# dynatrace-oss/index4j

Hardware: AMD Instinct MI355X
Metric: patterns/sec + LF-steps/sec, 1M x 8-char count() on 256 MiB log index (higher is better)
Workload: dtype int32; 1 GPU; count() batch of 1048576 random 8-char patterns per GPU on 256 MiB synthetic log text, sampleRate=32 (BASELINE.json configs[1]); 4 distinct batches rotate through the timed loop; image=expanded, text_chars=268435456, patterns_per_gpu=1048576, pattern_len=8, batches=4, count_checksum=151883111733, patterns_checked_vs_oracle=0, parallelism=dp1

## Files before the change

### include/fmx.h

```cpp
#ifndef FMX_H
#define FMX_H

#include <stddef.h>
#include <stdint.h>

#ifdef __cplusplus
extern "C" {
#endif

typedef struct fmx_index fmx_index;

#define FMX_OK 0
#define FMX_E_ARG (-1)
#define FMX_E_ALPHABET (-2)
#define FMX_E_FORMAT (-3)
#define FMX_E_VERSION (-4)
#define FMX_E_NO_DEVICE (-5)
#define FMX_E_HIP (-6)
#define FMX_E_NOMEM (-7)
#define FMX_E_UNSUPPORTED (-8)

#define FMX_ST_OK 0
#define FMX_ST_NOT_ENABLED 1
#define FMX_ST_POS_NEGATIVE 2
#define FMX_ST_STOP_TOO_LONG 3
#define FMX_ST_DEST_TOO_SMALL 4
#define FMX_ST_POS_TOO_LONG 5
#define FMX_ST_DEST_SIZE_ZERO 6
#define FMX_ST_NO_BOUNDARY 7
#define FMX_ST_DOES_NOT_FIT 8
#define FMX_ST_JAVA_AIOOBE 9
#define FMX_ST_TOO_MANY_RANGES 10


int fmx_build(const uint16_t *text, int32_t n, int32_t sample_rate, int enable_extract, fmx_index **out);
int fmx_build_on_device(const uint16_t *text, int32_t n, int32_t sample_rate, int enable_extract, int device,
                        fmx_index **out, int32_t *rounds, int64_t *rows_sorted, double *stage_seconds);
double fmx_build_wavelet_seconds(const fmx_index *idx);

int fmx_suffix_table_info(const fmx_index *idx, int32_t *chars, int64_t *bytes);

int fmx_window_cells_info(const fmx_index *idx, int64_t *bytes);
int fmx_locate_rows_info(const fmx_index *idx, int64_t *bytes, int64_t *replay_rows);
int fmx_resident_bytes(const fmx_index *idx, int64_t *image, int64_t *suffix_table, int64_t *window_directory);

int fmx_load(const uint8_t *ser, size_t len, fmx_index **out);

int fmx_save(const fmx_index *idx, int framed, uint8_t **buf, size_t *len);
int fmx_save_key_order_modelled(const fmx_index *idx);
void fmx_free_buffer(uint8_t *buf);
void fmx_free(fmx_index *idx);

int32_t fmx_input_length(const fmx_index *idx);
int32_t fmx_alphabet_length(const fmx_index *idx);
int32_t fmx_sample_rate(const fmx_index *idx);
int32_t fmx_extract_enabled(const fmx_index *idx);


int fmx_blob(const fmx_index *idx, const uint8_t **blob, size_t *len);
int fmx_to_device(fmx_index *idx, int device);
int fmx_attach_device_blob(void *device_blob, size_t len, int device, fmx_index **out);
void *fmx_device_blob(const fmx_index *idx, size_t *len);

// ... 282 lines not shown
```

### index4j_amd/_lib.py

```python
import ctypes as C
import os

_HERE = os.path.dirname(os.path.abspath(__file__))
LIB_PATH = os.environ.get("FMX_LIBRARY") or os.path.join(_HERE, "libfmx.so")

OK = 0
E_ARG, E_ALPHABET, E_FORMAT, E_VERSION, E_NO_DEVICE, E_HIP, E_NOMEM, E_UNSUPPORTED = -1, -2, -3, -4, -5, -6, -7, -8

ST_OK = 0
ST_NOT_ENABLED = 1
ST_POS_NEGATIVE = 2
ST_STOP_TOO_LONG = 3
ST_DEST_TOO_SMALL = 4
ST_POS_TOO_LONG = 5
ST_DEST_SIZE_ZERO = 6
ST_NO_BOUNDARY = 7
ST_DOES_NOT_FIT = 8
ST_JAVA_AIOOBE = 9
ST_TOO_MANY_RANGES = 10

SYMBOLS = [
    "fmx_build", "fmx_build_on_device", "fmx_build_wavelet_seconds", "fmx_suffix_table_info", "fmx_window_cells_info", "fmx_locate_rows_info", "fmx_load", "fmx_save", "fmx_save_key_order_modelled", "fmx_free_buffer", "fmx_free",
    "fmx_input_length", "fmx_alphabet_length", "fmx_sample_rate", "fmx_extract_enabled",
    "fmx_blob", "fmx_to_device", "fmx_attach_device_blob", "fmx_device_blob", "fmx_host_register", "fmx_host_unregister",
    "fmx_count_batch", "fmx_locate_batch", "fmx_locate_all_batch", "fmx_match_lines_batch", "fmx_match_query_batch", "fmx_count_class_batch", "fmx_locate_all_class_batch", "fmx_match_query_class_batch", "fmx_match_sequence_batch", "fmx_match_sequence_class_batch", "fmx_field_values_batch", "fmx_field_values_class_batch", "fmx_field_values_where_batch", "fmx_field_values_where_class_batch", "fmx_line_histogram_batch", "fmx_line_histogram_class_batch", "fmx_hit_histogram_where_batch", "fmx_hit_histogram_where_class_batch", "fmx_line_bounds_batch", "fmx_extract_packed_batch", "fmx_line_text_batch", "fmx_extract_packed_last_redo", "fmx_extract_batch", "fmx_extract_boundary_batch",
    "fmx_count_batch_dev", "fmx_count_plan_dev", "fmx_count_ordered_dev", "fmx_count_batch_is_planned", "fmx_batch_policy", "fmx_locate_batch_dev", "fmx_locate_all_ranges_dev", "fmx_locate_all_fill_dev", "fmx_line_table_build", "fmx_line_table_info", "fmx_line_bounds_batch_dev", "fmx_lines_of_hits_scratch_bytes", "fmx_lines_of_hits_dev", "fmx_hit_lines_geometry", "fmx_query_lines_scratch_bytes", "fmx_query_lines_of_hits_dev", "fmx_sequence_lines_scratch_bytes", "fmx_sequence_lines_of_hits_dev", "fmx_values_of_hits_scratch_bytes", "fmx_values_of_hits_dev", "fmx_values_fill_dev", "fmx_hits_in_lines_scratch_bytes", "fmx_hits_in_lines_dev", "fmx_lines_histogram_scratch_bytes", "fmx_hits_histogram_scratch_bytes", "fmx_lines_histogram_dev", "fmx_hits_histogram_dev", "fmx_class_ranges_scratch_bytes", "fmx_class_ranges_count_dev", "fmx_class_ranges_fill_dev", "fmx_class_hit_offsets_scratch_bytes", "fmx_class_hit_offsets_dev", "fmx_class_fold_status_dev", "fmx_extract_packed_scratch_bytes", "fmx_extract_packed_offsets_dev", "fmx_extract_packed_fill_dev", "fmx_extract_batch_dev", "fmx_extract_boundary_batch_dev",
    "fmx_locate_extract_batch", "fmx_locate_lines_batch", "fmx_locate_extract_batch_dev", "fmx_locate_lines_batch_dev",
    "fmx_count_segments", "fmx_locate_segments", "fmx_count_segments_dev", "fmx_locate_segments_dev", "fmx_count_locate_segments_dev",
    "fmx_count_locate_segments", "fmx_resident_bytes",
    "fmx_replicate", "fmx_device_of", "fmx_shard_range", "fmx_count_batch_multi", "fmx_locate_batch_multi", "fmx_extract_batch_multi",
    "fmx_extract_boundary_batch_multi", "fmx_count_locate_segments_multi", "fmx_count_batch_multi_dev",
    "fmx_count_locate_segments_multi_dev", "fmx_multi_synchronize",
    "fmx_wavelet_build", "fmx_wavelet_rank_batch", "fmx_wavelet_inverse_select_batch",
    "fmx_rrr_build", "fmx_rrr_rank_ones_batch", "fmx_rrr_access_batch", "fmx_rrr_rank_ones_batch_dev", "fmx_rrr_access_batch_dev",
    "fmx_sa_build", "fmx_sa_load", "fmx_sa_save", "fmx_sa_get", "fmx_sa_hash_code", "fmx_sa_count_batch", "fmx_sa_locate_batch",
    "fmx_sa_count_batch_dev", "fmx_sa_locate_batch_dev", "fmx_bwt",
    "fmx_convert_byte_pattern", "fmx_status_message", "fmx_status_kind", "fmx_last_error", "fmx_release_scratch", "fmx_device_count", "fmx_set_option",
    "fmx_synth_log", "fmx_synth_log_multichar", "fmx_synth_patterns",
]


def _load():
    if not os.path.exists(LIB_PATH):
        raise ImportError(
            "index4j_amd: %s is missing - build it with `python -c 'import __graft_entry__ as g; g.build()'` "
            "or `make -C index4j_amd/csrc` (hipcc, gfx950). There is no CPU fallback." % LIB_PATH
        )
    L = C.CDLL(LIB_PATH)
    vp, i32, u16, u64 = C.c_void_p, C.c_int32, C.c_uint16, C.c_uint64
    P = C.POINTER
    sz = C.c_size_t
    L.fmx_build.argtypes = [vp, i32, i32, C.c_int, P(vp)]
    L.fmx_build_on_device.argtypes = [vp, i32, i32, C.c_int, C.c_int, P(vp), P(i32), P(C.c_int64), P(C.c_double)]
    L.fmx_build_wavelet_seconds.argtypes = [vp]
    L.fmx_build_wavelet_seconds.restype = C.c_double
    L.fmx_suffix_table_info.argtypes = [vp, P(i32), P(C.c_int64)]
    L.fmx_window_cells_info.argtypes = [vp, P(C.c_int64)]
    L.fmx_locate_rows_info.argtypes = [vp, P(C.c_int64), P(C.c_int64)]
    L.fmx_load.argtypes = [vp, sz, P(vp)]
    L.fmx_save.argtypes = [vp, C.c_int, P(vp), P(sz)]
    L.fmx_save_key_order_modelled.argtypes = [vp]
    L.fmx_batch_policy.argtypes = [vp, C.c_int, C.c_int64]
    L.fmx_free_buffer.argtypes = [vp]
    L.fmx_free_buffer.restype = None
    L.fmx_free.argtypes = [vp]
    L.fmx_free.restype = None
    for name in ("fmx_input_length", "fmx_alphabet_length", "fmx_sample_rate", "fmx_extract_enabled"):
        getattr(L, name).argtypes = [vp]
        getattr(L, name).restype = i32
    L.fmx_blob.argtypes = [vp, P(vp), P(sz)]
    L.fmx_to_device.argtypes = [vp, C.c_int]
    L.fmx_attach_device_blob.argtypes = [vp, sz, C.c_int, P(vp)]
    L.fmx_device_blob.argtypes = [vp, P(sz)]
    L.fmx_device_blob.restype = vp
    L.fmx_host_register.argtypes = [vp, sz]
    L.fmx_host_unregister.argtypes = [vp]
    L.fmx_count_batch.argtypes = [vp, vp, vp, i32, vp, vp, vp]
    L.fmx_locate_batch.argtypes = [vp, vp, vp, i32, i32, vp, i32, vp, vp, vp]
    L.fmx_extract_batch.argtypes = [vp, vp, vp, i32, vp, i32, i32, vp, vp, vp]
# ... 150 lines not shown
```

### index4j_amd/csrc/fmx_api.cpp

```cpp
#include "../../include/fmx.h"
#include "fmx_device.hpp"
#include "fmx_build_stage.hpp"
#include "fmx_hit_values.hpp"
#include "fmx_model.hpp"
#include "fmx_options.hpp"
#include "fmx_plan.hpp"
#include "fmx_sa_index.hpp"

#include <hip/hip_runtime.h>

#include <immintrin.h>

#include <atomic>
#include <chrono>
#include <climits>
#include <condition_variable>
#include <deque>
#include <cstdio>
#include <cstdlib>
#include <cstring>
#include <map>
#include <memory>
#include <mutex>
#include <new>
// ... 1216 lines not shown
    if (key_bits == 8 && idx->hdr.wt_sigma <= fmx::kOrder1MaxSigma &&
        fmx::order1_lds_bytes(fmx::kPlanDefaultBins, idx->hdr.wt_sigma) <= fmx::kPlanCodesLdsMax) {
        void *d_o1 = nullptr;
        const size_t bytes = (size_t)idx->hdr.wt_sigma * idx->hdr.wt_sigma * 2 * sizeof(float);
        if (hipMalloc(&d_o1, bytes) == hipSuccess) {
            if (k_launch_suffix_order1(idx, idx->dev, static_cast<float *>(d_o1), nullptr) == 0 &&
                hipStreamSynchronize(nullptr) == hipSuccess) {
                idx->d_suffix_order1 = d_o1;
                idx->dev.suffix_order1 = static_cast<const float *>(d_o1);
            } else {
                (void)hipFree(d_o1);
            }
        }
    }
}

int fmx_suffix_table_info(const fmx_index *idx, int32_t *chars, int64_t *bytes) {
    return guarded([&]() -> int {
    if (!idx || idx->sa) return fail(FMX_E_ARG, "not an FM-index handle");
    if (chars) *chars = idx->dev.suffix_table ? idx->dev.suffix_chars : 0;
    if (bytes) *bytes = (int64_t)idx->suffix_table_bytes;
    return FMX_OK;
    });
}

int fmx_blob(const fmx_index *idx_c, const uint8_t **blob, size_t *len) {
    return guarded([&]() -> int {
    fmx_index *idx = const_cast<fmx_index *>(idx_c);
    if (!idx || !blob || !len) return fail(FMX_E_ARG, "null argument");
    int rc = ensure_blob(idx);
    if (rc) return rc;
    *blob = idx->blob.data();
    *len = idx->blob.size();
    return FMX_OK;
    });
}

int fmx_to_device(fmx_index *idx, int device) {
    return guarded([&]() -> int {
    if (!idx) return fail(FMX_E_ARG, "null index");
    if (idx->sa) {
        std::string err;
        const int rc = fmx::sa_to_device(*idx->sa, device, err);
        return rc ? fail(rc, err) : FMX_OK;
    }
    int rc = ensure_blob(idx);
// ... 3000 lines not shown
```

### index4j_amd/csrc/fmx_kernels.hip

```cpp
#include <atomic>
#include <cstring>

#include <hip/hip_runtime.h>

#include "fmx_device.hpp"
#include "fmx_options.hpp"
#include "fmx_plan.hpp"

#if !defined(FMX_KNS)
#define FMX_KNS fmx
#endif

namespace FMX_KNS {
using namespace fmx;
#include "fmx_kernel_api.hpp"

#if FMX_COMPACT
#define FMX_KERNEL(BLOCK) __global__ __launch_bounds__(BLOCK)
#else
#define FMX_KERNEL(BLOCK) __global__ __launch_bounds__(BLOCK) __attribute__((amdgpu_waves_per_eu(8, 8)))
#endif
#ifndef FMX_WALK_WAVES
#define FMX_WALK_WAVES 8
#endif
// ... 1402 lines not shown
template <int kBlock>
FMX_KERNEL(kBlock) void k_rrr_access(DevIndex ix, const int32_t *__restrict__ positions, int32_t n,
                                     uint8_t *__restrict__ out, int32_t *__restrict__ status_out) {
    __shared__ uint16_t s_inv[kInvEntries];
    stage_inverse_table(s_inv, ix.inv_global);
    const RrrView v = rrr_view_from(Quad{ix.sampled.off_rec, ix.sampled.off_bits, (uint32_t)ix.sampled.length, (uint32_t)ix.sampled.total_ones});
    const int64_t stride = (int64_t)gridDim.x * kBlock;
    for (int64_t q = (int64_t)blockIdx.x * kBlock + threadIdx.x; q < n; q += stride) {
        int status = ST_OK;
        const bool bit = rrr_access(ix.base, v, s_inv, positions[q], status);
        out[q] = status ? 0 : (bit ? 1 : 0);
        if (status_out) status_out[q] = status;
    }
}



struct PlanTables {
    const int16_t *s_map;
    const float2 *s_o1;
    const int32_t *s_c;
    bool o1;
    int sigma, below, fine_shift, bins;
};
__device__ __forceinline__ bool plan_uses_order1(const DevIndex &ix, const SortShape &sh, int code_bits, int bins, size_t extra_lds) {
    return code_bits == 8 && sh.sa_key == 2 && ix.suffix_order1 != nullptr && ix.wt_sigma <= kOrder1MaxSigma &&
           order1_lds_bytes(bins, ix.wt_sigma) + extra_lds <= kPlanCodesLdsMax;
}
__device__ __forceinline__ PlanTables plan_tables_stage(const DevIndex &ix, const SortShape &sh, int16_t *s_map, uint32_t *after, bool o1) {
    PlanTables t;
    t.sigma = ix.wt_sigma;
    t.bins = 1 << sh.coarse_bits;
    t.below = sh.total_bits - sh.coarse_bits;
    t.fine_shift = t.below > 8 ? t.below - 8 : 0;
    t.o1 = o1;
    for (int i = threadIdx.x; i < 256; i += kTileThreads) s_map[i] = ix.char2code[i];
    float2 *s_o1 = reinterpret_cast<float2 *>(after);
    int32_t *s_c = reinterpret_cast<int32_t *>(s_o1 + (o1 ? t.sigma * t.sigma : 0));
    if (o1) {
        const float2 *src = reinterpret_cast<const float2 *>(ix.suffix_order1);
        for (int i = threadIdx.x; i < t.sigma * t.sigma; i += kTileThreads) s_o1[i] = src[i];
        for (int i = threadIdx.x; i <= t.sigma; i += kTileThreads) s_c[i] = i < ix.n_c ? ix.C[i] : ix.length;
    }
    t.s_map = s_map;
    t.s_o1 = s_o1;
    t.s_c = s_c;
    return t;
}

template <int kCodeBits>
__device__ __forceinline__ Quad plan_record(const DevIndex &ix, const PlanTables &L, const SortShape &sh, const uint16_t *__restrict__ pat,
                                            int32_t beg, int32_t m, const TailWords &tail, uint32_t &bin) {
    const int sigma = L.sigma;
    uint32_t ch[8];
    pattern_tail_chars(tail, pat, beg, m, ch);
    const uint64_t word = pattern_code_word<kCodeBits>(ix, L.s_map, ch, m);
    uint32_t key;
    if (sh.sa_key) {
        key = 0;
        constexpr uint32_t cmask = (1u << kCodeBits) - 1u;
        const int32_t c_last = (int32_t)(word & cmask);
        if (m > 0 && c_last != 0) {
            int32_t start = ix.C[c_last], end = 0, back = 0;
            int len = fm_suffix_len(ix, m);
            if (len > 64 / kCodeBits) len = 64 / kCodeBits;
            if (len >= 2 && kCodeBits == ix.suffix_key_bits && sh.sa_key == 1) {
                const int bits = len * kCodeBits;
                const uint64_t tk = bits >= 64 ? word : (word & ((1ull << bits) - 1ull));
                if ((uint32_t)(tk >> (bits - kCodeBits)) != 0u && tk != kSuffixEmpty) (void)fm_suffix_lookup(ix, tk, len, start, end, back);
            } else if (len >= 2 && L.o1) {
                auto code_at = [&](int j) { return (uint32_t)(word >> (j * kCodeBits)) & cmask; };
                uint32_t x = code_at(len - 1), y = code_at(len - 2);
                if (x >= (uint32_t)sigma) x = 0;
                if (y >= (uint32_t)sigma) y = 0;
                float lo = (float)L.s_c[x ? x : ((uint32_t)c_last < (uint32_t)sigma ? c_last : 0)], width = 0.0f;
                if (x != 0 && y != 0) {
                    float2 fp = L.s_o1[x * sigma + y];
                    if (fp.y > 0.0f) {
                        const float nx = (float)(L.s_c[x + 1] - L.s_c[x]);
                        lo = (float)L.s_c[x] + fp.x * nx;
                        width = fp.y * nx;
                        for (int j = len - 3; j >= 0 && width >= 1.0f; --j) {
                            x = y;
                            y = code_at(j);
                            if (y == 0 || y >= (uint32_t)sigma) break;
                            fp = L.s_o1[x * sigma + y];
                            if (fp.y <= 0.0f) break;
                            lo += width * fp.x;
                            width *= fp.y;
                        }
                    }
                }
                start = (int32_t)lo;
                if (start < 0) start = 0;
                if (start > ix.length) start = ix.length;
            } else if (len >= 2 && kCodeBits == ix.suffix_key_bits) {
                auto code_at = [&](int j) { return (uint32_t)(word >> (j * kCodeBits)) & cmask; };
                uint32_t x = code_at(len - 1), y = code_at(len - 2);
                float lo = (float)ix.C[x ? x : c_last], width = 0.0f;
                int32_t s2 = 0, e2 = 0;
                if (x != 0 && y != 0 && fm_suffix_lookup(ix, (uint64_t)y | ((uint64_t)x << kCodeBits), 2, s2, e2, back)) {
                    lo = (float)s2;
                    width = (float)(e2 - s2);
                    for (int j = len - 3; j >= 0 && width >= 1.0f; --j) {
                        x = y;
                        y = code_at(j);
                        if (y == 0 || !fm_suffix_lookup(ix, (uint64_t)y | ((uint64_t)x << kCodeBits), 2, s2, e2, back)) break;
                        const float cx = (float)ix.C[x], nx = (float)(ix.C[x + 1] - ix.C[x]);
                        lo += width * ((float)s2 - cx) / nx;
                        width *= (float)(e2 - s2) / nx;
                    }
                }
                start = (int32_t)lo;
                if (start < 0) start = 0;
                if (start > ix.length) start = ix.length;
            }
            key = (uint32_t)start;
        }
    } else {
        key = suffix_key(word, kCodeBits, sh.chars, sh.bits);
    }
    const uint32_t lenf = m < 0 ? 0u : ((uint32_t)m < kPlanLongPattern ? (uint32_t)m : kPlanLongPattern);
    Quad q;
    q.x = (uint32_t)word;
    q.y = (uint32_t)(word >> 32);
    q.z = key;
    q.w = lenf | (((key >> L.fine_shift) & ((1u << kFineBits) - 1u)) << 22);
    uint32_t c = key >> L.below;
    if (c >= (uint32_t)L.bins) c = (uint32_t)L.bins - 1u;
    bin = c;
    return q;
}

template <int kCodeBits>
__global__ __launch_bounds__(kTileThreads) void k_plan_codes(DevIndex ix, const uint16_t *__restrict__ pat,
                                                             const int32_t *__restrict__ pat_off, int32_t n,
                                                             SortShape sh, PlanRec *__restrict__ recs,
                                                             uint32_t *__restrict__ ghist, uint32_t *__restrict__ mixed,
                                                             uint32_t epoch) {
    extern __shared__ uint32_t s_hist[];
    __shared__ int16_t s_map[256];
    const int bins = 1 << sh.coarse_bits;
    for (int i = threadIdx.x; i < bins; i += kTileThreads) s_hist[i] = 0;
    const PlanTables L = plan_tables_stage(ix, sh, s_map, s_hist + bins, plan_uses_order1(ix, sh, kCodeBits, bins, 0));
    __syncthreads();
    const int64_t base = (int64_t)blockIdx.x * kTile;
    const int32_t m_first = pat_off[1] - pat_off[0];
    bool differs = false;
    constexpr int kGroup = kTileItems < 4 ? kTileItems : 4;
    for (int k0 = 0; k0 < kTileItems; k0 += kGroup) {
        int32_t beg[kGroup], len[kGroup];
        TailWords tail[kGroup];
#pragma unroll
        for (int k = 0; k < kGroup; ++k) {
            const int64_t p = base + (int64_t)(k0 + k) * kTileThreads + threadIdx.x;
            beg[k] = 0;
            len[k] = -1;
            if (p < n) {
                beg[k] = pat_off[p];
                len[k] = pat_off[p + 1] - beg[k];
            }
        }
#pragma unroll
        for (int k = 0; k < kGroup; ++k) tail[k] = pattern_tail_load(pat, beg[k], len[k]);
#pragma unroll
        for (int k = 0; k < kGroup; ++k) {
            const int64_t p = base + (int64_t)(k0 + k) * kTileThreads + threadIdx.x;
            if (p >= n) continue;
            differs |= len[k] != m_first;
            uint32_t c;
// ... 281 lines not shown
        for (int k = 0; k < 8; ++k) {
            const int i = i0 + k * kTileThreads + (int)threadIdx.x;
            if (cnt[k]) s_cnt[i] = s_scan[i] + got[k];
        }
    }
    __syncthreads();
#pragma unroll
    for (int k = 0; k < kTileItems; ++k) {
        uint32_t slot = 0;
        if constexpr (kFromRange) slot = wave_ticket(&s_cnt[0], bin[k] == 0u);
        if (bin[k] != 0xffffffffu && !(kFromRange && bin[k] == 0u)) slot = atomicAdd(&s_cnt[bin[k]], 1u);
        if (bin[k] != 0xffffffffu) *reinterpret_cast<Quad *>(recs_out + slot) = mine[k];
    }
    __syncthreads();
    if (threadIdx.x == 0) s_last = atomicAdd(ticket, 1u) == gridDim.x - 1 ? 1u : 0u;
    __syncthreads();
    if (s_last) {
        for (int i = threadIdx.x; i < bins; i += kTileThreads) {
            ghist[i] = 0;
            cursor[i] = 0;
        }
        if (threadIdx.x == 0) *ticket = 0;
    }
}

__global__ __launch_bounds__(kFineThreads) void k_plan_fine(PlanRec *__restrict__ recs, int32_t n) {
    constexpr int n_bins = 1 << kFineBits;
    __shared__ uint32_t s_bin[n_bins];
    __shared__ Quad s_rec[kFineWindow];
    for (int i = threadIdx.x; i < n_bins; i += kFineThreads) s_bin[i] = 0;
    __syncthreads();
    const int64_t base = (int64_t)blockIdx.x * kFineWindow;
    Quad r[kFineItems];
    uint32_t bin[kFineItems];
#pragma unroll
    for (int k = 0; k < kFineItems; ++k) {
        const int64_t q = base + (int64_t)k * kFineThreads + threadIdx.x;
        bin[k] = 0xffffffffu;
        if (q < n) {
            r[k] = ld_quad(recs + q);
            bin[k] = r[k].w >> 22;
            r[k].w &= kPlanLongPattern;
        }
    }
#pragma unroll
    for (int k = 0; k < kFineItems; ++k)
// ... 165 lines not shown
    if (options().plan_fused && !fine_pass && n_cu > 0 && tiles <= n_cu) {
        const size_t lds_fused = std::max(lds_codes, (size_t)bins * 8);
        const uint32_t spin_limit = (uint32_t)options().plan_spin_limit.load();
        if (code_bits == 8)
            hipLaunchKernelGGL(k_plan_fused<8>, dim3(tiles), dim3(kTileThreads), lds_fused, st, ix, pat, off, n, sh, ordered, ghist, ticket,
                               ticket + 2, epoch, spin_limit);
        else if (code_bits == 12)
            hipLaunchKernelGGL(k_plan_fused<12>, dim3(tiles), dim3(kTileThreads), (size_t)bins * 8, st, ix, pat, off, n, sh, ordered, ghist,
                               ticket, ticket + 2, epoch, spin_limit);
        else
            hipLaunchKernelGGL(k_plan_fused<16>, dim3(tiles), dim3(kTileThreads), (size_t)bins * 8, st, ix, pat, off, n, sh, ordered, ghist,
                               ticket, ticket + 2, epoch, spin_limit);
    } else {
    if (code_bits == 8)
        hipLaunchKernelGGL(k_plan_codes<8>, dim3(tiles), dim3(kTileThreads), lds_codes, st, ix, pat, off, n, sh, recs,
                           ghist, ticket + 2, epoch);
    else if (code_bits == 12)
        hipLaunchKernelGGL(k_plan_codes<12>, dim3(tiles), dim3(kTileThreads), (size_t)bins * 4, st, ix, pat, off, n, sh, recs,
                           ghist, ticket + 2, epoch);
    else
        hipLaunchKernelGGL(k_plan_codes<16>, dim3(tiles), dim3(kTileThreads), (size_t)bins * 4, st, ix, pat, off, n, sh, recs,
                           ghist, ticket + 2, epoch);
    if (hipError_t e = hipGetLastError(); e != hipSuccess) return (int)e;
    hipLaunchKernelGGL(k_plan_scatter<false>, dim3(tiles), dim3(kTileThreads), (size_t)bins * 8, st, recs, nullptr, nullptr, 0, n, bins,
                       sh.total_bits - sh.coarse_bits, ghist, cursor, ticket, ordered);
    }
    if (options().plan_fine == 2 || (options().plan_fine == 1 && !sh.sa_key))
        hipLaunchKernelGGL(k_plan_fine, dim3((n + kFineWindow - 1) / kFineWindow), dim3(kFineThreads), 0, st, ordered, n);
    plan->recs = ordered;
    plan->redo_list = reinterpret_cast<int32_t *>(recs);
    plan->redo_count = ticket + 8;
    plan->mixed = ticket + 2;
    plan->epoch = epoch;
    plan->n = n;
    plan->code_bits = code_bits;
    plan->shape = sh;
    plan->look_up = ix.look_up;
    plan->sigma = ix.wt_sigma;
    return (int)hipGetLastError();
}

int launch_count(const DevIndex &ix, int n_cu, const uint16_t *pat, const int32_t *off, const CountPlan *plan,
                 bool plan_is_foreign, int32_t n, int32_t *counts, int32_t *lf, int32_t *status, int32_t *range,
                 hipStream_t st) {
    if (n <= 0) return 0;
    const PlanRec *recs = (plan && plan->recs && plan->n == n) ? static_cast<const PlanRec *>(plan->recs) : nullptr;
    CountPlan none;
    const CountPlan &pl = recs ? *plan : none;
// ... 134 lines not shown
    if (n <= 0) return 0;
    const int32_t slots = fm_locate_slots(max_matches, loc_cap);
    const PlanRec *order = nullptr;
    const uint32_t *order_idle = nullptr;
    const size_t need = (ix.rows && !options().rows_order.load()) ? 0 : walk_workspace_bytes(ix, n);
    if (workspace && need != 0 && workspace_bytes >= need && loc_cap > 0) {
        uint8_t *wsb = static_cast<uint8_t *>(workspace);
        uint32_t *ghist = reinterpret_cast<uint32_t *>(wsb);
        uint32_t *cursor = ghist + (1 << kCoarseBitsMax);
        uint32_t *ticket = cursor + (1 << kCoarseBitsMax);
        PlanRec *ordered = reinterpret_cast<PlanRec *>(wsb + kPlanHeadBytes);
        if (!head_is_zero) {
            hipError_t e = hipMemsetAsync(workspace, 0, kPlanHeadBytes, st);
            if (e != hipSuccess) return (int)e;
        }
        int total_bits = 1;
        while (total_bits < 32 && (1ll << total_bits) <= (long long)ix.length) ++total_bits;
        const int coarse_bits = total_bits < options().coarse_bits ? total_bits : (int)options().coarse_bits;
        const int bins = (1 << coarse_bits) + 1, below = total_bits - coarse_bits;
        const int tiles = (n + kTile - 1) / kTile;
        hipLaunchKernelGGL(k_walk_hist, dim3(tiles), dim3(kTileThreads), (size_t)bins * 4, st, range, n, bins, below, taken,
                           max_matches, ghist, nullptr, nullptr, 1);
        if (hipError_t e = hipGetLastError(); e != hipSuccess) return (int)e;
        hipLaunchKernelGGL(k_plan_scatter<true>, dim3(tiles), dim3(kTileThreads), (size_t)bins * 8, st, nullptr, range, taken,
                           max_matches, n, bins, below, ghist, cursor, ticket, ordered);
        if (hipError_t e = hipGetLastError(); e != hipSuccess) return (int)e;
        if (options().walk_fine)
            hipLaunchKernelGGL(k_plan_fine, dim3((n + kFineWindow - 1) / kFineWindow), dim3(kFineThreads), 0, st, ordered, n);
        order = ordered;
        order_idle = ticket + 1;
    }
    if (ix.rows) {
        const int32_t lanes_log2 = fm_rows_lanes_log2(slots);
        FMX_DISPATCH(k_locate_rows, (int64_t)n << lanes_log2, ix, range, n, max_matches, locs, loc_cap, lanes_log2, found, lf, status, taken,
                     order, set_locs, set_base);
        return (int)hipGetLastError();
    }
    const int64_t tickets = (int64_t)n * fm_walk_lanes(slots);
    if (ix.win && options().walk_queue.load() && ix.sample_rate >= 4 && slots >= options().walk_queue_min_slots.load()) {
        const int64_t waves = (tickets + 63) / 64;
        int32_t per = options().walk_queue.load();
        const int32_t chunk = 64 * per;
        int32_t burst = options().walk_burst.load();
        if (burst <= 0) burst = ix.sample_rate / 4 > 2 ? ix.sample_rate / 4 : 2;
        (void)waves;
        FMX_DISPATCH_FORM(k_locate_walk_q, ix, (tickets + per - 1) / per, ix, range, n, max_matches, locs, loc_cap, slots, found, lf, status, taken, order,
                     order_idle, set_locs, set_base, chunk, burst);
        return (int)hipGetLastError();
// ... 88 lines not shown
    const int order_min = options().boundary_order_min;
    if (order_min <= 0 || n < order_min || n > INT32_MAX) return 0;
    return kPlanHeadBytes + (size_t)n * sizeof(PlanRec) + 64;
}

static int launch_position_order(const DevIndex &ix, const int32_t *positions, int32_t n, const int32_t *slot_found, int32_t slots,
                                 void *order_ws, bool head_is_zero, PlanRec *ordered, hipStream_t st) {
    uint8_t *wsb = static_cast<uint8_t *>(order_ws);
    uint32_t *ghist = reinterpret_cast<uint32_t *>(wsb);
    uint32_t *cursor = ghist + (1 << kCoarseBitsMax);
    uint32_t *ticket = cursor + (1 << kCoarseBitsMax);
    if (!head_is_zero) {
        hipError_t e = hipMemsetAsync(order_ws, 0, kPlanHeadBytes, st);
        if (e != hipSuccess) return (int)e;
    }
    int total_bits = 1;
    while (total_bits < 32 && (1ll << total_bits) <= (long long)ix.length) ++total_bits;
    const int coarse_bits = total_bits < options().coarse_bits ? total_bits : (int)options().coarse_bits;
    const int bins = (1 << coarse_bits) + 1, below = total_bits - coarse_bits;
    const int tiles = (n + kTile - 1) / kTile;
    hipLaunchKernelGGL(k_walk_hist, dim3(tiles), dim3(kTileThreads), (size_t)bins * 4, st, nullptr, n, bins, below, nullptr, 0, ghist,
                       positions, slot_found, slots < 1 ? 1 : slots);
    if (hipError_t e = hipGetLastError(); e != hipSuccess) return (int)e;
    hipLaunchKernelGGL(k_plan_scatter<true>, dim3(tiles), dim3(kTileThreads), (size_t)bins * 8, st, nullptr, nullptr, nullptr, 0, n, bins,
                       below, ghist, cursor, ticket, ordered, positions, slot_found, slots < 1 ? 1 : slots);
    if (hipError_t e = hipGetLastError(); e != hipSuccess) return (int)e;
    hipLaunchKernelGGL(k_plan_fine, dim3((n + kFineWindow - 1) / kFineWindow), dim3(kFineThreads), 0, st, ordered, n);
    return (int)hipGetLastError();
}

int launch_extract(const DevIndex &ix, int n_cu, const int32_t *start, const int32_t *stop, int64_t n, uint16_t *dst,
                   int32_t dst_len, int32_t offset, int32_t *out_len, int32_t *lf, int32_t *status,
                   const int32_t *slot_found, int32_t slots, int32_t fixed_len, void *order_ws, size_t order_ws_bytes,
                   bool head_is_zero, hipStream_t st) {
    if (n <= 0) return 0;
    const PlanRec *order = nullptr;
    const size_t order_need = slot_found ? boundary_order_bytes(ix, n) : 0;
    if (order_ws && order_need != 0 && order_ws_bytes >= order_need) {
        PlanRec *ordered = reinterpret_cast<PlanRec *>(static_cast<uint8_t *>(order_ws) + kPlanHeadBytes);
        if (int e = launch_position_order(ix, start, (int32_t)n, slot_found, slots, order_ws, head_is_zero, ordered, st)) return e;
        order = ordered;
    }
    FMX_DISPATCH_WIN(k_extract, ix, n, ix, start, stop, n, dst, dst_len, offset, out_len, lf, status, slot_found, slots, fixed_len, order);
    return (int)hipGetLastError();
}

struct BoundaryShape {
    int block, group, accel;
// ... 156 lines not shown
```

### index4j_amd/csrc/fmx_options.cpp

```cpp
#include "fmx_options.hpp"

#include <string_view>

#include "fmx_model.hpp"

namespace fmx {
namespace {

bool is_block(int v) { return v == 512 || v == 1024; }
bool is_boundary_group(int v) { return v == 0 || v == 1 || v == 2 || v == 4 || v == 8 || v == 16; }
bool is_first_fill(int v) { return v == 0 || v == 2; }
bool is_entry_bytes(int v) { return v == 0 || v == 4 || v == 6; }
bool is_fence_count(int v) { return v >= 0 && v <= 32768 && !(v & (v - 1)); }

using O = Options;
constexpr Accept any = range(INT_MIN, INT_MAX);

constexpr OptionRow kOptions[] = {
    {"block", 512, &O::block, one_of(is_block), "threads per workgroup"},
    {"groups_per_cu", 16, &O::groups_per_cu, range(1, 64), "grid cap: workgroups per CU, the rest grid-stride"},
    {"lds_pad_kb", 0, &O::lds_pad_kb, range(0, 96), "experiment knob: extra dynamic LDS per workgroup (lowers occupancy)"},

    {"sort_min", 16384, &O::sort_min, at_least(0), "batches at least this large are processed in suffix-sorted order (0 = never)"},
    {"sort_bits", 28, &O::sort_bits, range(1, 32), "full key width: floor(sort_bits / bits-per-code) trailing characters"},
// ... 51 lines not shown
    {"host_pipeline_chunk", 262144, &O::host_pipeline_chunk, at_least(65536), "patterns per stage of that pipeline"},
    {"host_mapped", 1, &O::host_mapped, flag(), "every array of a host-buffer count registered -> one launch over the mapped arrays, no copies"},
    {"host_direct_stores", 1, &O::host_direct_stores, flag(), "the pipeline's kernels store results straight into registered arrays"},
    {"host_stage_threads", 0, &O::host_stage_threads, range(0, 64), "host threads that stage a pageable array into pinned memory (0 / 1 = the runtime's own staging)"},

    {"segments_direct", 1, &O::segments_direct, flag(), "0 = every segment's hits staged and appended (A/B)"},
    {"segments_overlap", 1, &O::segments_overlap, flag(), "0 = a segment set's kernels all on the caller's stream (A/B)"},
    {"segments_overlap_min", 262144, &O::segments_overlap_min, at_least(0), "... and only for batches at least this large"},
};
static_assert(sizeof(kOptions) / sizeof(kOptions[0]) == 58, "a new option needs its entry in tests/test_option_ranges.py too");

}

Options::Options() {
    for (const OptionRow &row : kOptions)
        if (row.store.member) (this->*row.store.member).store(row.def);
}

Options &options() {
    static Options instance;
    return instance;
}

const OptionRow *find_option(const char *name) {
    for (const OptionRow &row : kOptions)
        if (std::string_view(row.name) == name) return &row;
    return nullptr;
}

bool OptionRow::set(int value) const {
    if (value < accept.lo || value > accept.hi || (accept.one_of && !accept.one_of(value))) return false;
    if (accept.flag) value = value != 0;
    if (store.member)
        (options().*store.member).store(value);
    else
        store.setter(value);
    return true;
}

}
```

### index4j_amd/csrc/fmx_options.hpp

```cpp
#pragma once

#include <atomic>
#include <climits>

namespace fmx {

constexpr int kCoarseBitsMax = 14;

struct Options {
    std::atomic<int> block, groups_per_cu, lds_pad_kb;
    std::atomic<int> sort_min, sort_bits, coarse_bits, plan_fine, plan_sa_key, plan_sa_min, plan_min_per_string, plan_fused,
        plan_spin_limit, code_bits_12, suffix_table, regroup_by_length, lf_steps_executed_only, count_halve_uniform, count_lean;
    std::atomic<int> walk_pack, walk_queue, walk_queue_min_slots, walk_burst, walk_order_min, walk_fine, rows_order;
    std::atomic<int> boundary_accel, boundary_group, boundary_first_fill, boundary_narrow, boundary_narrow_min, boundary_rounds,
        boundary_order_min;
    std::atomic<int> sb_cache_limit, suffix_table_mb, suffix_table_chars, suffix_table_image_fraction, window_cells,
        window_cells_mb, window_entry_bytes, window_flat_fraction, locate_rows, sa_fences, sa_fence_chars, wavelet_on_device;
    std::atomic<int> host_small_max, host_pipeline_min, host_pipeline_chunk, host_mapped, host_direct_stores, host_stage_threads,
        segments_direct, segments_overlap, segments_overlap_min;
    Options();
};
Options &options();

struct Accept {
    int lo, hi;
    bool flag;
    bool (*one_of)(int);
};
constexpr Accept range(int lo, int hi) { return {lo, hi, false, nullptr}; }
constexpr Accept at_least(int lo) { return {lo, INT_MAX, false, nullptr}; }
constexpr Accept flag() { return {INT_MIN, INT_MAX, true, nullptr}; }
constexpr Accept one_of(bool (*pred)(int)) { return {INT_MIN, INT_MAX, false, pred}; }

struct Store {
    std::atomic<int> Options::*member = nullptr;
    void (*setter)(int) = nullptr;
    constexpr Store(std::atomic<int> Options::*m) : member(m) {}
    constexpr Store(void (*s)(int)) : setter(s) {}
};

struct OptionRow {
    const char *name;
    int def;
    Store store;
    Accept accept;
// ... 7 lines not shown
```

Before: 8.893 billion patterns/s.

## Stage plan scatter in LDS by bin to write coalesced runs

Adds k_plan_scatter_runs, which sorts each tile's records by coarse bin in shared memory and then writes them out in contiguous runs instead of scattering each record to global memory on its own. It is selected by default when the large dynamic LDS allocation can be granted, and falls back to the old kernel otherwise. It also changes the plan chain's early-exit test to a fine-bin boundary check with float slack, and moves the m_first read into shared memory. The new kernel trades much higher LDS use, and so lower occupancy, for better write coalescing. The changed loop-exit test may run more or fewer LF steps per pattern.

```diff
diff --git a/include/fmx.h b/include/fmx.h
--- a/include/fmx.h
+++ b/include/fmx.h
@@ -39,6 +39,9 @@
 double fmx_build_wavelet_seconds(const fmx_index *idx);
 
 int fmx_suffix_table_info(const fmx_index *idx, int32_t *chars, int64_t *bytes);
+
+int fmx_plan_scatter_runs(int on);
+int fmx_plan_scatter_info(int64_t *runs, int64_t *plain);
 
 int fmx_window_cells_info(const fmx_index *idx, int64_t *bytes);
 int fmx_locate_rows_info(const fmx_index *idx, int64_t *bytes, int64_t *replay_rows);
diff --git a/index4j_amd/_lib.py b/index4j_amd/_lib.py
--- a/index4j_amd/_lib.py
+++ b/index4j_amd/_lib.py
@@ -20,7 +20,7 @@
 ST_TOO_MANY_RANGES = 10
 
 SYMBOLS = [
-    "fmx_build", "fmx_build_on_device", "fmx_build_wavelet_seconds", "fmx_suffix_table_info", "fmx_window_cells_info", "fmx_locate_rows_info", "fmx_load", "fmx_save", "fmx_save_key_order_modelled", "fmx_free_buffer", "fmx_free",
+    "fmx_build", "fmx_build_on_device", "fmx_build_wavelet_seconds", "fmx_suffix_table_info", "fmx_plan_scatter_runs", "fmx_plan_scatter_info", "fmx_window_cells_info", "fmx_locate_rows_info", "fmx_load", "fmx_save", "fmx_save_key_order_modelled", "fmx_free_buffer", "fmx_free",
     "fmx_input_length", "fmx_alphabet_length", "fmx_sample_rate", "fmx_extract_enabled",
     "fmx_blob", "fmx_to_device", "fmx_attach_device_blob", "fmx_device_blob", "fmx_host_register", "fmx_host_unregister",
     "fmx_count_batch", "fmx_locate_batch", "fmx_locate_all_batch", "fmx_match_lines_batch", "fmx_match_query_batch", "fmx_count_class_batch", "fmx_locate_all_class_batch", "fmx_match_query_class_batch", "fmx_match_sequence_batch", "fmx_match_sequence_class_batch", "fmx_field_values_batch", "fmx_field_values_class_batch", "fmx_field_values_where_batch", "fmx_field_values_where_class_batch", "fmx_line_histogram_batch", "fmx_line_histogram_class_batch", "fmx_hit_histogram_where_batch", "fmx_hit_histogram_where_class_batch", "fmx_line_bounds_batch", "fmx_extract_packed_batch", "fmx_line_text_batch", "fmx_extract_packed_last_redo", "fmx_extract_batch", "fmx_extract_boundary_batch",
@@ -55,6 +55,8 @@
     L.fmx_build_wavelet_seconds.argtypes = [vp]
     L.fmx_build_wavelet_seconds.restype = C.c_double
     L.fmx_suffix_table_info.argtypes = [vp, P(i32), P(C.c_int64)]
+    L.fmx_plan_scatter_runs.argtypes = [C.c_int]
+    L.fmx_plan_scatter_info.argtypes = [P(C.c_int64), P(C.c_int64)]
     L.fmx_window_cells_info.argtypes = [vp, P(C.c_int64)]
     L.fmx_locate_rows_info.argtypes = [vp, P(C.c_int64), P(C.c_int64)]
     L.fmx_load.argtypes = [vp, sz, P(vp)]
diff --git a/index4j_amd/csrc/fmx_api.cpp b/index4j_amd/csrc/fmx_api.cpp
--- a/index4j_amd/csrc/fmx_api.cpp
+++ b/index4j_amd/csrc/fmx_api.cpp
@@ -1262,6 +1262,14 @@
     if (bytes) *bytes = (int64_t)idx->suffix_table_bytes;
     return FMX_OK;
     });
+}
+
+int fmx_plan_scatter_runs(int on) { return fmx::plan_scatter_stats().want_runs.exchange(on != 0 ? 1 : 0); }
+
+int fmx_plan_scatter_info(int64_t *runs, int64_t *plain) {
+    if (runs) *runs = (int64_t)fmx::plan_scatter_stats().runs.load();
+    if (plain) *plain = (int64_t)fmx::plan_scatter_stats().plain.load();
+    return FMX_OK;
 }
 
 int fmx_blob(const fmx_index *idx_c, const uint8_t **blob, size_t *len) {
diff --git a/index4j_amd/csrc/fmx_kernels.hip b/index4j_amd/csrc/fmx_kernels.hip
--- a/index4j_amd/csrc/fmx_kernels.hip
+++ b/index4j_amd/csrc/fmx_kernels.hip
@@ -1448,6 +1448,7 @@
     const int32_t *s_c;
     bool o1;
     int sigma, below, fine_shift, bins;
+    float cut_slack;
 };
 __device__ __forceinline__ bool plan_uses_order1(const DevIndex &ix, const SortShape &sh, int code_bits, int bins, size_t extra_lds) {
     return code_bits == 8 && sh.sa_key == 2 && ix.suffix_order1 != nullptr && ix.wt_sigma <= kOrder1MaxSigma &&
@@ -1460,6 +1461,11 @@
     t.below = sh.total_bits - sh.coarse_bits;
     t.fine_shift = t.below > 8 ? t.below - 8 : 0;
     t.o1 = o1;
+    {
+        const uint32_t top = (uint32_t)ix.length + ((uint32_t)ix.length >> 16) + 1u;
+        const int most = ix.suffix_chars < 64 / 8 ? ix.suffix_chars : 64 / 8;
+        t.cut_slack = (float)(most > 2 ? most - 2 : 0) * ldexpf(1.0f, (31 - __clz((int)(top | 1u))) - 24);
+    }
     for (int i = threadIdx.x; i < 256; i += kTileThreads) s_map[i] = ix.char2code[i];
     float2 *s_o1 = reinterpret_cast<float2 *>(after);
     int32_t *s_c = reinterpret_cast<int32_t *>(s_o1 + (o1 ? t.sigma * t.sigma : 0));
@@ -1472,6 +1478,11 @@
     t.s_o1 = s_o1;
     t.s_c = s_c;
     return t;
+}
+
+__device__ __forceinline__ bool plan_chain_open(const PlanTables &L, float lo, float width) {
+    const float hi = lo + width + L.cut_slack;
+    return ((uint32_t)lo >> L.fine_shift) != ((uint32_t)hi >> L.fine_shift);
 }
 
 template <int kCodeBits>
@@ -1506,7 +1517,7 @@
                         const float nx = (float)(L.s_c[x + 1] - L.s_c[x]);
                         lo = (float)L.s_c[x] + fp.x * nx;
                         width = fp.y * nx;
-                        for (int j = len - 3; j >= 0 && width >= 1.0f; --j) {
+                        for (int j = len - 3; j >= 0 && plan_chain_open(L, lo, width); --j) {
                             x = y;
                             y = code_at(j);
                             if (y == 0 || y >= (uint32_t)sigma) break;
@@ -1528,7 +1539,7 @@
                 if (x != 0 && y != 0 && fm_suffix_lookup(ix, (uint64_t)y | ((uint64_t)x << kCodeBits), 2, s2, e2, back)) {
                     lo = (float)s2;
                     width = (float)(e2 - s2);
-                    for (int j = len - 3; j >= 0 && width >= 1.0f; --j) {
+                    for (int j = len - 3; j >= 0 && plan_chain_open(L, lo, width); --j) {
                         x = y;
                         y = code_at(j);
                         if (y == 0 || !fm_suffix_lookup(ix, (uint64_t)y | ((uint64_t)x << kCodeBits), 2, s2, e2, back)) break;
@@ -1566,12 +1577,14 @@
                                                              uint32_t epoch) {
     extern __shared__ uint32_t s_hist[];
     __shared__ int16_t s_map[256];
+    __shared__ int32_t s_m_first;
     const int bins = 1 << sh.coarse_bits;
     for (int i = threadIdx.x; i < bins; i += kTileThreads) s_hist[i] = 0;
+    if (threadIdx.x == 0) s_m_first = pat_off[1] - pat_off[0];
     const PlanTables L = plan_tables_stage(ix, sh, s_map, s_hist + bins, plan_uses_order1(ix, sh, kCodeBits, bins, 0));
     __syncthreads();
     const int64_t base = (int64_t)blockIdx.x * kTile;
-    const int32_t m_first = pat_off[1] - pat_off[0];
+    const int32_t m_first = s_m_first;
     bool differs = false;
     constexpr int kGroup = kTileItems < 4 ? kTileItems : 4;
     for (int k0 = 0; k0 < kTileItems; k0 += kGroup) {
@@ -1899,6 +1912,194 @@
         }
         if (threadIdx.x == 0) *ticket = 0;
     }
+}
+
+constexpr int kRunsScanPer = 8;
+constexpr size_t kPlanRunsLdsMax = (160u << 10) - 256;
+constexpr size_t plan_runs_lds_bytes(int bins) { return (size_t)kTile * (sizeof(Quad) + 4) + (size_t)bins * 12; }
+template <bool kFromRange>
+__global__ __launch_bounds__(kTileThreads) void k_plan_scatter_runs(const PlanRec *__restrict__ recs_in,
+                                                                    const int32_t *__restrict__ range,
+                                                                    const int32_t *__restrict__ taken, int32_t max_matches,
+                                                                    int32_t n, int bins, int below,
+                                                                    uint32_t *__restrict__ ghist,
+                                                                    uint32_t *__restrict__ cursor,
+                                                                    uint32_t *__restrict__ ticket,
+                                                                    PlanRec *__restrict__ recs_out,
+                                                                    const int32_t *__restrict__ froms = nullptr,
+                                                                    const int32_t *__restrict__ slot_found = nullptr,
+                                                                    int32_t slots = 1) {
+    const int fine_shift = below > 8 ? below - 8 : 0;
+    extern __shared__ __align__(16) uint8_t s_runs[];
+    __shared__ uint32_t s_wave[2][kTileThreads / 64];
+    __shared__ uint32_t s_last;
+    Quad *s_rec = reinterpret_cast<Quad *>(s_runs);
+    uint32_t *s_slot = reinterpret_cast<uint32_t *>(s_rec + kTile);
+    uint32_t *s_scan = s_slot + kTile, *s_cnt = s_scan + bins, *s_first = s_cnt + bins;
+    if (kFromRange && blockIdx.x == 0 && threadIdx.x == 0) ticket[1] = ghist[0];
+    for (int i = threadIdx.x; i < bins; i += kTileThreads) s_cnt[i] = 0;
+    __syncthreads();
+    const int64_t base = (int64_t)blockIdx.x * kTile;
+    Quad mine[kTileItems];
+    uint32_t bin[kTileItems], rank[kTileItems];
+#pragma unroll
+    for (int k = 0; k < kTileItems; ++k) {
+        const int64_t p = base + (int64_t)k * kTileThreads + threadIdx.x;
+        bin[k] = 0xffffffffu;
+        if (p < n) {
+            if constexpr (kFromRange) {
+                const int2 r = walk_pair(range, froms, slot_found, slots, p);
+                mine[k].x = (uint32_t)r.x;
+                mine[k].y = (uint32_t)r.y;
+                mine[k].z = walk_key(r.x, r.y, taken, max_matches, p);
+                mine[k].w = ((mine[k].z >> fine_shift) & ((1u << kFineBits) - 1u)) << 22;
+                bin[k] = walk_bin(mine[k].z, below, bins);
+            } else {
+                mine[k] = ld_quad(recs_in + p);
+                uint32_t c = mine[k].z >> below;
+                if (c >= (uint32_t)bins) c = (uint32_t)bins - 1u;
+                bin[k] = c;
+            }
+            mine[k].z = (uint32_t)p;
+        }
+    }
+#pragma unroll
+    for (int k = 0; k < kTileItems; ++k) {
+        rank[k] = 0;
+        if constexpr (kFromRange) rank[k] = wave_ticket(&s_cnt[0], bin[k] == 0u);
+        if (bin[k] != 0xffffffffu && !(kFromRange && bin[k] == 0u)) rank[k] = atomicAdd(&s_cnt[bin[k]], 1u);
+    }
+    const int per = (bins + kTileThreads - 1) / kTileThreads;
+    const int lo = (int)threadIdx.x * per;
+    const int lane = threadIdx.x & 63, wave = threadIdx.x >> 6;
+    uint32_t g[kRunsScanPer], c[kRunsScanPer];
+    uint32_t gsum = 0, csum = 0;
+#pragma unroll
+    for (int k = 0; k < kRunsScanPer; ++k) {
+        g[k] = (k < per && lo + k < bins) ? ghist[lo + k] : 0u;
+        gsum += g[k];
+    }
+    uint32_t gincl = gsum;
+    for (int d = 1; d < 64; d <<= 1) {
+        const uint32_t t = __shfl_up(gincl, d);
+        if (lane >= d) gincl += t;
+    }
+    if (lane == 63) s_wave[0][wave] = gincl;
+    __syncthreads();
+    uint32_t before = 0;
+    for (int w = 0; w < wave; ++w) before += s_wave[0][w];
+    uint32_t run = before + gincl - gsum;
+#pragma unroll
+    for (int k = 0; k < kRunsScanPer; ++k) {
+        if (k < per && lo + k < bins) {
+            s_scan[lo + k] = run;
+            c[k] = s_cnt[lo + k];
+        } else {
+            c[k] = 0u;
+        }
+        run += g[k];
+        csum += c[k];
+    }
+    uint32_t cincl = csum;
+    for (int d = 1; d < 64; d <<= 1) {
+        const uint32_t t = __shfl_up(cincl, d);
+        if (lane >= d) cincl += t;
+    }
+    if (lane == 63) s_wave[1][wave] = cincl;
+    __syncthreads();
+    before = 0;
+    for (int w = 0; w < wave; ++w) before += s_wave[1][w];
+    run = before + cincl - csum;
+#pragma unroll
+    for (int k = 0; k < kRunsScanPer; ++k) {
+        if (k < per && lo + k < bins) s_first[lo + k] = run;
+        run += c[k];
+    }
+    for (int i0 = 0; i0 < bins; i0 += kTileThreads * 8) {
+        uint32_t got[8], cnt[8];
+#pragma unroll
+        for (int k = 0; k < 8; ++k) {
+            const int i = i0 + k * kTileThreads + (int)threadIdx.x;
+            cnt[k] = i < bins ? s_cnt[i] : 0u;
+            got[k] = cnt[k] ? atomicAdd(&cursor[i], cnt[k]) : 0u;
+        }
+#pragma unroll
+        for (int k = 0; k < 8; ++k) {
+            const int i = i0 + k * kTileThreads + (int)threadIdx.x;
+            if (cnt[k]) s_cnt[i] = s_scan[i] + got[k];
+        }
+    }
+    __syncthreads();
+    uint32_t turn = 0;
+    if (threadIdx.x == 0) turn = atomicAdd(ticket, 1u);
+#pragma unroll
+    for (int k = 0; k < kTileItems; ++k) {
+        if (bin[k] == 0xffffffffu) continue;
+        const uint32_t at = s_first[bin[k]] + rank[k];
+        s_rec[at] = mine[k];
+        s_slot[at] = s_cnt[bin[k]] + rank[k];
+    }
+    if (threadIdx.x == 0) s_last = turn == gridDim.x - 1 ? 1u : 0u;
+    __syncthreads();
+    const int64_t left = (int64_t)n - base;
+    const int held = left < kTile ? (int)left : kTile;
+#pragma unroll
+    for (int k = 0; k < kTileItems; ++k) {
+        const int j = k * kTileThreads + (int)threadIdx.x;
+        if (j < held) *reinterpret_cast<Quad *>(recs_out + s_slot[j]) = s_rec[j];
+    }
+    if (s_last) {
+        for (int i = threadIdx.x; i < bins; i += kTileThreads) {
+            ghist[i] = 0;
+            cursor[i] = 0;
+        }
+        if (threadIdx.x == 0) *ticket = 0;
+    }
+}
+
+constexpr int kRunsDevices = 64;
+template <bool kFromRange>
+static std::atomic<int> &plan_scatter_runs_granted(int dev) {
+    static std::atomic<int> granted[kRunsDevices];
+    return granted[dev];
+}
+template <bool kFromRange>
+static bool plan_scatter_takes_runs(int bins, int &dev) {
+    if (!plan_scatter_stats().want_runs.load()) return false;
+    const size_t lds = plan_runs_lds_bytes(bins);
+    if (lds > kPlanRunsLdsMax || (bins + kTileThreads - 1) / kTileThreads > kRunsScanPer) return false;
+    if (hipGetDevice(&dev) != hipSuccess || dev < 0 || dev >= kRunsDevices) return false;
+    std::atomic<int> &granted = plan_scatter_runs_granted<kFromRange>(dev);
+    int have = granted.load();
+    if (have == 0) {
+        int most = 0;
+        const bool fits = hipDeviceGetAttribute(&most, hipDeviceAttributeMaxSharedMemoryPerBlock, dev) == hipSuccess &&
+                          (size_t)most >= kPlanRunsLdsMax + 256;
+        const bool ok = fits && hipFuncSetAttribute(reinterpret_cast<const void *>(&k_plan_scatter_runs<kFromRange>),
+                                                    hipFuncAttributeMaxDynamicSharedMemorySize, (int)kPlanRunsLdsMax) == hipSuccess;
+        if (!ok) (void)hipGetLastError();
+        have = ok ? 1 : -1;
+        granted.store(have);
+    }
+    return have == 1;
+}
+template <bool kFromRange>
+static void launch_plan_scatter(int tiles, hipStream_t st, const PlanRec *recs_in, const int32_t *range, const int32_t *taken,
+                                int32_t max_matches, int32_t n, int bins, int below, uint32_t *ghist, uint32_t *cursor,
+                                uint32_t *ticket, PlanRec *recs_out, const int32_t *froms, const int32_t *slot_found, int32_t slots) {
+    int dev = 0;
+    if (plan_scatter_takes_runs<kFromRange>(bins, dev)) {
+        hipLaunchKernelGGL(k_plan_scatter_runs<kFromRange>, dim3(tiles), dim3(kTileThreads), plan_runs_lds_bytes(bins), st, recs_in, range,
+                           taken, max_matches, n, bins, below, ghist, cursor, ticket, recs_out, froms, slot_found, slots);
+        if (hipGetLastError() == hipSuccess) {
+            plan_scatter_stats().runs.fetch_add(1);
+            return;
+        }
+        plan_scatter_runs_granted<kFromRange>(dev).store(-1);
+    }
+    hipLaunchKernelGGL(k_plan_scatter<kFromRange>, dim3(tiles), dim3(kTileThreads), (size_t)bins * 8, st, recs_in, range, taken,
+                       max_matches, n, bins, below, ghist, cursor, ticket, recs_out, froms, slot_found, slots);
+    plan_scatter_stats().plain.fetch_add(1);
 }
 
 __global__ __launch_bounds__(kFineThreads) void k_plan_fine(PlanRec *__restrict__ recs, int32_t n) {
@@ -2110,8 +2311,8 @@
         hipLaunchKernelGGL(k_plan_codes<16>, dim3(tiles), dim3(kTileThreads), (size_t)bins * 4, st, ix, pat, off, n, sh, recs,
                            ghist, ticket + 2, epoch);
     if (hipError_t e = hipGetLastError(); e != hipSuccess) return (int)e;
-    hipLaunchKernelGGL(k_plan_scatter<false>, dim3(tiles), dim3(kTileThreads), (size_t)bins * 8, st, recs, nullptr, nullptr, 0, n, bins,
-                       sh.total_bits - sh.coarse_bits, ghist, cursor, ticket, ordered);
+    launch_plan_scatter<false>(tiles, st, recs, nullptr, nullptr, 0, n, bins, sh.total_bits - sh.coarse_bits, ghist, cursor, ticket, ordered,
+                               nullptr, nullptr, 1);
     }
     if (options().plan_fine == 2 || (options().plan_fine == 1 && !sh.sa_key))
         hipLaunchKernelGGL(k_plan_fine, dim3((n + kFineWindow - 1) / kFineWindow), dim3(kFineThreads), 0, st, ordered, n);
@@ -2292,8 +2493,8 @@
         hipLaunchKernelGGL(k_walk_hist, dim3(tiles), dim3(kTileThreads), (size_t)bins * 4, st, range, n, bins, below, taken,
                            max_matches, ghist, nullptr, nullptr, 1);
         if (hipError_t e = hipGetLastError(); e != hipSuccess) return (int)e;
-        hipLaunchKernelGGL(k_plan_scatter<true>, dim3(tiles), dim3(kTileThreads), (size_t)bins * 8, st, nullptr, range, taken,
-                           max_matches, n, bins, below, ghist, cursor, ticket, ordered);
+        launch_plan_scatter<true>(tiles, st, nullptr, range, taken, max_matches, n, bins, below, ghist, cursor, ticket, ordered, nullptr,
+                                  nullptr, 1);
         if (hipError_t e = hipGetLastError(); e != hipSuccess) return (int)e;
         if (options().walk_fine)
             hipLaunchKernelGGL(k_plan_fine, dim3((n + kFineWindow - 1) / kFineWindow), dim3(kFineThreads), 0, st, ordered, n);
@@ -2428,8 +2629,8 @@
     hipLaunchKernelGGL(k_walk_hist, dim3(tiles), dim3(kTileThreads), (size_t)bins * 4, st, nullptr, n, bins, below, nullptr, 0, ghist,
                        positions, slot_found, slots < 1 ? 1 : slots);
     if (hipError_t e = hipGetLastError(); e != hipSuccess) return (int)e;
-    hipLaunchKernelGGL(k_plan_scatter<true>, dim3(tiles), dim3(kTileThreads), (size_t)bins * 8, st, nullptr, nullptr, nullptr, 0, n, bins,
-                       below, ghist, cursor, ticket, ordered, positions, slot_found, slots < 1 ? 1 : slots);
+    launch_plan_scatter<true>(tiles, st, nullptr, nullptr, nullptr, 0, n, bins, below, ghist, cursor, ticket, ordered, positions, slot_found,
+                              slots < 1 ? 1 : slots);
     if (hipError_t e = hipGetLastError(); e != hipSuccess) return (int)e;
     hipLaunchKernelGGL(k_plan_fine, dim3((n + kFineWindow - 1) / kFineWindow), dim3(kFineThreads), 0, st, ordered, n);
     return (int)hipGetLastError();
diff --git a/index4j_amd/csrc/fmx_options.cpp b/index4j_amd/csrc/fmx_options.cpp
--- a/index4j_amd/csrc/fmx_options.cpp
+++ b/index4j_amd/csrc/fmx_options.cpp
@@ -97,6 +97,11 @@
     return instance;
 }
 
+PlanScatterStats &plan_scatter_stats() {
+    static PlanScatterStats instance;
+    return instance;
+}
+
 const OptionRow *find_option(const char *name) {
     for (const OptionRow &row : kOptions)
         if (std::string_view(row.name) == name) return &row;
diff --git a/index4j_amd/csrc/fmx_options.hpp b/index4j_amd/csrc/fmx_options.hpp
--- a/index4j_amd/csrc/fmx_options.hpp
+++ b/index4j_amd/csrc/fmx_options.hpp
@@ -21,6 +21,12 @@
     Options();
 };
 Options &options();
+
+struct PlanScatterStats {
+    std::atomic<int> want_runs{1};
+    std::atomic<long long> runs{0}, plain{0};
+};
+PlanScatterStats &plan_scatter_stats();
 
 struct Accept {
     int lo, hi;
```

After: 8.984 billion patterns/s (median of 6 runs). 1.0% higher.
